# yabebalFantaye/MCEvidence

Hardware: AMD Instinct MI355X
Metric: knn_queries_per_sec (higher is better)
Workload: dtype f16 filter + f64 refine (exact f64 results)

## Files before the change

include/mcevidence_hip.h:

```cpp
#ifndef MCEVIDENCE_HIP_H
#define MCEVIDENCE_HIP_H

#include <stddef.h>
#include <stdint.h>

#ifdef __cplusplus
extern "C" {
#endif

#define MCE_ABI_VERSION 3

#define MCE_OK 0
#define MCE_ERR_INVALID (-1)
#define MCE_ERR_K_RANGE (-2)
#define MCE_ERR_HIP (-3)
#define MCE_ERR_NO_DEVICE (-4)
#define MCE_ERR_WORKSPACE (-5)
#define MCE_ERR_DIM_RANGE (-6)
#define MCE_ERR_VERIFY (-7)

#define MCE_MAX_K 32
#define MCE_MAX_DIM 63
#define MCE_GENERIC_MAX_K 1024
#define MCE_GENERIC_MAX_DIM 1024
// ... 286 lines not shown
                            double* d_fs, double* out, void* ws, size_t ws_bytes, void* stream);

int mce_set_prune_mode(int mode);
int mce_get_prune_mode(void);

int mce_set_sym_mode(int mode);
int mce_get_sym_mode(void);
int mce_last_prune_stats(double *chunk_fraction, double *tile_fraction);

void mce_set_profiling(int on);
double mce_last_kernel_ms(void);
int mce_last_search_stats(double* out, int32_t n);

int mce_debug_mfma_tile_f16(const uint16_t* yprime, const uint16_t* xprime, int32_t kst, float* out, int32_t device);
int mce_debug_mfma_tiles_f16(const uint16_t* yprime, const uint16_t* xprime, int32_t kst, int32_t ntiles, float* out, int32_t device);

#ifdef __cplusplus
}
#endif
#endif
```

mcevidence_amd/_capi.py:

```python
from __future__ import annotations

import ctypes
import os
import sys

import numpy as np

_HERE = os.path.dirname(os.path.abspath(__file__))
LIB_PATH = os.environ.get("MCE_LIB") or os.path.join(_HERE, "libmcevidence_hip.so")

MCE_OK = 0
MCE_ERR_INVALID = -1
MCE_ERR_K_RANGE = -2
MCE_ERR_HIP = -3
MCE_ERR_NO_DEVICE = -4
MCE_ERR_WORKSPACE = -5
MCE_ERR_DIM_RANGE = -6
MCE_ERR_VERIFY = -7
MCE_MAX_K = 32
MCE_MAX_DIM = 63
SELF_NONE, SELF_INCLUDE, SELF_EXCLUDE = 0, 1, 2

_c = ctypes
_P = _c.c_void_p
# ... 5 lines not shown
    "mce_last_verify_rows": (_c.c_int32, []),
    "mce_source_hash": (_c.c_char_p, []),
    "mce_release_device_memory": (None, []),
    "mce_set_search_mode": (_c.c_int, [_c.c_int]),
    "mce_get_search_mode": (_c.c_int, []),
    "mce_set_prune_mode": (_c.c_int, [_c.c_int]),
    "mce_get_prune_mode": (_c.c_int, []),
    "mce_set_sym_mode": (_c.c_int, [_c.c_int]),
    "mce_get_sym_mode": (_c.c_int, []),
    "mce_last_prune_stats": (_c.c_int, [_c.POINTER(_c.c_double), _c.POINTER(_c.c_double)]),
    "mce_set_profiling": (None, [_c.c_int]),
    "mce_last_kernel_ms": (_c.c_double, []),
    "mce_last_search_stats": (_c.c_int, [_c.c_void_p, _c.c_int32]),
    "mce_debug_mfma_tile_f16": (_c.c_int, [_P, _P, _c.c_int32, _P, _c.c_int32]),
    "mce_debug_mfma_tiles_f16": (_c.c_int, [_P, _P, _c.c_int32, _c.c_int32, _P, _c.c_int32]),
    "mce_options_push": (_c.c_int, [_P]),
    "mce_options_pop": (_c.c_int, []),
    "mce_knn_f64_opt": (_c.c_int, [_P, _c.c_int64, _P, _c.c_int64, _c.c_int32, _c.c_int32, _c.c_int32, _c.c_int64, _P, _P, _c.c_int32, _P]),
    "mce_knn_dotp_f64_opt": (_c.c_int, [_P, _c.c_int64, _P, _c.c_int64, _c.c_int32, _c.c_int32, _c.c_int32, _c.c_int64, _P, _P, _P, _P, _P, _c.c_int32, _P]),
    "mce_knn_dotp_f64_dev_opt": (_c.c_int, [_P, _c.c_int64, _P, _c.c_int64, _c.c_int32, _c.c_int32, _c.c_int32, _c.c_int64, _P, _P, _P, _P, _P, _c.c_size_t, _P, _P]),
    "mce_knn_workspace_bytes_opt": (_c.c_size_t, [_c.c_int64, _c.c_int64, _c.c_int32, _c.c_int32, _P]),
    "mce_knn_f64": (_c.c_int, [_P, _c.c_int64, _P, _c.c_int64, _c.c_int32, _c.c_int32, _c.c_int32, _c.c_int64, _P, _P, _c.c_int32]),
    "mce_dotp_f64": (_c.c_int, [_P, _c.c_int64, _c.c_int32, _c.c_int32, _c.c_int32, _c.c_int32, _P, _P, _P, _c.c_int32]),
    "mce_knn_dotp_f64": (_c.c_int, [_P, _c.c_int64, _P, _c.c_int64, _c.c_int32, _c.c_int32, _c.c_int32, _c.c_int64, _P, _P, _P, _P, _P, _c.c_int32]),
    "mce_evidence_feed_f64": (_c.c_int, [_P, _c.c_int64, _c.c_int64, _P, _c.c_int64, _c.c_int64, _c.c_int32, _c.c_int32, _c.c_int32,
                                         _P, _P, _P, _P, _P, _c.c_int32]),
    "mce_evidence_feed_part_f64": (_c.c_int, [_P, _c.c_int64, _c.c_int64, _P, _c.c_int64, _c.c_int64, _c.c_int32, _c.c_int32, _c.c_int32,
                                              _P, _P, _c.c_int32, _c.c_int32, _P, _P, _P, _P, _c.c_int32]),
    "mce_evidence_feed_whiten_f64": (_c.c_int, [_P, _c.c_int64, _c.c_int64, _c.c_int32, _c.c_int32, _P, _P, _P, _P, _P, _c.POINTER(_c.c_double), _P,
                                                _c.POINTER(_c.c_uint64), _c.c_int32]),
# ... 1112 lines not shown
    if y.shape != x.shape or y.shape[0] != 32 or y.shape[1] % 16 or not 1 <= y.shape[1] // 16 <= 8:
        raise ValueError("yprime and xprime must be float16 [32, 16*kst], kst = 1..8")
    out = np.empty((32, 32), dtype=np.float32)
    check(load().mce_debug_mfma_tile_f16(y.ctypes.data, x.ctypes.data, y.shape[1] // 16, out.ctypes.data, int(device)))
    return out


def debug_mfma_tiles(yprime, xprime, device=0):
    y = np.ascontiguousarray(yprime, dtype=np.float16)
    x = np.ascontiguousarray(xprime, dtype=np.float16)
    if y.ndim != 3 or y.shape != x.shape or y.shape[1] != 32 or y.shape[2] % 16 or not 1 <= y.shape[2] // 16 <= 8:
        raise ValueError("yprime and xprime must be float16 [ntiles, 32, 16*kst], kst = 1..8")
    out = np.empty((y.shape[0], 32, 32), dtype=np.float32)
    check(load().mce_debug_mfma_tiles_f16(y.ctypes.data, x.ctypes.data, y.shape[2] // 16, y.shape[0], out.ctypes.data, int(device)))
    return out
```

mcevidence_amd/csrc/capi_common.hpp:

```cpp
#pragma once
namespace {

thread_local char g_err[512] = "";
thread_local char g_last_kernel[256] = "";
thread_local int g_prof_on = 0;
thread_local std::vector<std::pair<hipEvent_t, hipEvent_t>> g_ev_pool;
thread_local size_t g_ev_used = 0;
thread_local size_t g_ev_calls = 0;
thread_local bool g_in_tail = false;
thread_local int g_split_depth = 0;
thread_local double g_last_prune_geom[3] = {0, 0, 0};
thread_local double g_last_flops_main = 0.0, g_last_flops_all = 0.0;
thread_local std::vector<std::pair<hipEvent_t, hipEvent_t>> g_evs_pool;
thread_local size_t g_evs_used = 0;

int fail(int code, const char* fmt, ...)
{
    va_list ap;
    va_start(ap, fmt);
    vsnprintf(g_err, sizeof(g_err), fmt, ap);
    va_end(ap);
    return code;
}

#define MCE_HIP(call)                                                                              \
    do {                                                                                           \
        hipError_t e_ = (call);                                                                    \
        if (e_ != hipSuccess)                                                                      \
            return fail(MCE_ERR_HIP, "%s failed: %s (%s:%d)", #call, hipGetErrorString(e_), __FILE__, __LINE__); \
    } while (0)

std::atomic<int> g_mode{0};
std::atomic<int> g_prune_mode{0};
struct Tuning {
    bool sym_kernel_f16 = false, tail_split = true, prune_prof = false, wide = true;
    int spin_limit = 1 << 21, sym_bucket = 0, sym_panel = 0, sym_seed_rows = 0, sym_seed_share = 2, sym_seed_mode = -1;
    int f16_seed_rows = -1, f16_seed_share = -1, f16_seed_tg = -1, rsplit = 0, panel_debug = 0, sym_chains = 0;
    size_t feed_wave_bytes = 0;
};
Tuning read_tuning()
{
    Tuning t;
    auto num = [](const char* name, int dflt) { const char* e = getenv(name); return e ? atoi(e) : dflt; };
    const char* e = getenv("MCE_SYM_KERNEL");
    t.sym_kernel_f16 = e && strcmp(e, "f16") == 0;
    t.spin_limit = num("MCE_SYM_SPIN_LIMIT", 1 << 21);
    t.sym_bucket = num("MCE_SYM_BUCKET", 0);
    t.sym_panel = num("MCE_SYM_PANEL", 0);
    t.sym_chains = num("MCE_SYM_CHAINS", 0);
    t.sym_seed_rows = num("MCE_SYM_SEED_ROWS", 0);
    t.sym_seed_share = num("MCE_SYM_SEED_SHARE", 2);
    t.sym_seed_mode = num("MCE_SYM_SEED_MODE", -1);
    t.f16_seed_rows = num("MCE_F16_SEED_ROWS", -1);
    t.f16_seed_share = num("MCE_F16_SEED_SHARE", -1);
    t.f16_seed_tg = num("MCE_F16_SEED_TG", -1);
    t.rsplit = num("MCE_RSPLIT", 0);
    t.tail_split = num("MCE_TAIL_SPLIT", 1) != 0;
    t.wide = num("MCE_WIDE", 1) != 0;
    t.panel_debug = num("MCE_PANEL_DEBUG", 0);
    t.prune_prof = getenv("MCE_PRUNE_PROF") != nullptr;
// ... 180 lines not shown
```

mcevidence_amd/csrc/capi_debug.hpp:

```cpp
#pragma once

namespace mce {
template <int KST>
__global__ __launch_bounds__(64) void mfma_tile_probe_kernel(const _Float16* __restrict__ yp, const _Float16* __restrict__ xp, float* __restrict__ out)
{
    const int lane = threadIdx.x;
    yp += (size_t)blockIdx.x * 32 * 16 * KST;
    xp += (size_t)blockIdx.x * 32 * 16 * KST;
    out += (size_t)blockIdx.x * 1024;
    v16f acc = {0.f, 0.f, 0.f, 0.f, 0.f, 0.f, 0.f, 0.f, 0.f, 0.f, 0.f, 0.f, 0.f, 0.f, 0.f, 0.f};
#pragma unroll
    for (int ks = 0; ks < KST; ++ks) {
        const v8h a = *reinterpret_cast<const v8h*>(yp + (lane & 31) * (16 * KST) + 16 * ks + 8 * (lane >> 5));
        const v8h b = *reinterpret_cast<const v8h*>(xp + (lane & 31) * (16 * KST) + 16 * ks + 8 * (lane >> 5));
        acc = __builtin_amdgcn_mfma_f32_32x32x16_f16(a, b, acc, 0, 0, 0);
    }
#pragma unroll
    for (int r = 0; r < 16; ++r) out[((r & 3) + 8 * (r >> 2) + 4 * (lane >> 5)) * 32 + (lane & 31)] = acc[r];
}
}

extern "C" int mce_debug_mfma_tiles_f16(const uint16_t* yprime, const uint16_t* xprime, int32_t kst, int32_t ntiles, float* out, int32_t device)
{
    if (!yprime || !xprime || !out) return fail(MCE_ERR_INVALID, "null pointer argument");
// ... 23 lines not shown
            case 7: hipLaunchKernelGGL(mce::mfma_tile_probe_kernel<7>, g, dim3(64), 0, nullptr, y, x, o); break;
            default: hipLaunchKernelGGL(mce::mfma_tile_probe_kernel<8>, g, dim3(64), 0, nullptr, y, x, o); break;
        }
        e = hipGetLastError();
    }
    if (e == hipSuccess) e = hipMemcpy(out, dout, (size_t)ntiles * 1024 * sizeof(float), hipMemcpyDeviceToHost);
    (void)hipFree(dy); (void)hipFree(dx); (void)hipFree(dout);
    if (e != hipSuccess) return fail(MCE_ERR_HIP, "mfma tile probe: %s", hipGetErrorString(e));
    return MCE_OK;
}

extern "C" int mce_debug_mfma_tile_f16(const uint16_t* yprime, const uint16_t* xprime, int32_t kst, float* out, int32_t device)
{
    return mce_debug_mfma_tiles_f16(yprime, xprime, kst, 1, out, device);
}
```

mcevidence_amd/csrc/capi_plan.hpp:

```cpp
#pragma once
namespace {

using mce::kMaxDevices;
constexpr int kAssumedCUs = 256;

size_t align_up(size_t x, size_t a) { return (x + a - 1) / a * a; }

constexpr bool kPruneHeavyDefault = false;
constexpr int kPruneHeavyMinBlocks = 64, kPruneHeavyCount = 700, kPruneHeavyMaxShare = 16, kPruneHeavyMinCount = 32, kPruneHeavyMaxRounds = 60;
constexpr double kPruneHeavyFullRounds = 10.0;
constexpr int kPruneHeavySplit = 4, kPruneHeavyMaxSplit = 8;
constexpr int kPruneWaveQueries = mce::kHQT * 32;
constexpr int kWideMinBlocks = 480;
bool prune_heavy_enabled()
{
    if (t_no_heavy) return false;
    const char* e = env_prune_heavy();
    return kPruneHeavyDefault || (e && *e && strcmp(e, "0") != 0);
}
static_assert(mce::kPruneWavesPerBlock == mce::kHWaves, "prune.hip orders kHWaves waves per query block");

constexpr int kRefineMargin = 2;
struct Plan {
    const mce::KnnVariant* v = nullptr;
// ... 10 lines not shown
    int64_t nrow_pad = 0;
    int nqblk = 0;
    int64_t nq_pad = 0;
    int rsplit = 1;
    int L = 4;
    size_t off_yf = 0, off_pd = 0, off_pi = 0, off_center = 0, off_msum = 0, total = 0;
    double cost = 0.0;
    int ksel = 0;
    bool twopass = false;
    bool wide_ok = false;
    bool prune = false;
    bool kd_ready = false;
    int part = 0, nparts = 1;
    int sym_qb_lo = 0, sym_qb_hi = 0;
    bool apo = false;
    int apo_phase = 0;
    int apo_nsplit = 1;
    int apo_panel = 0;
    int64_t pl_nr = 0;
    mce::PruneLayout pl;
    size_t off_prune = 0;
    size_t off_heavy = 0;
    int heavy_max = 0;
    bool sym = false;
    bool sym_active = false;
    mce::SymLayout sl;
    size_t off_sym = 0;
    int sym_nsplit = 1;
    int sym_panel = 0;
};
// ... 299 lines not shown
```

mcevidence_amd/csrc/capi_search.hpp:

```cpp
#pragma once
namespace {

double ln_unit_ball(int d) { return 0.5 * d * std::log(M_PI) - std::lgamma(1.0 + 0.5 * d); }

hipError_t launch_sym_merge(int KCAP, double* pd, int* pi, int64_t nq_pad, const mce::SymParams& sym, int qb_lo, int qb_hi, hipStream_t st, int stride = 1)
{
    const int nb = qb_hi > qb_lo ? (qb_hi - qb_lo + stride - 1) / stride : 0;
    if (nb <= 0) return hipSuccess;
    const dim3 g((unsigned)nb), b(mce::kSymMergeThreads);
    static_assert(mce::kSymMergeThreads == mce::f16_qpb(4), "one merge block per query block");
    switch (KCAP) {
        case 4: hipLaunchKernelGGL(mce::sym_merge_kernel<4>, g, b, 0, st, pd, pi, nq_pad, sym.bucket_cnt, sym.bucket_flag, sym.bucket, sym.cap, qb_lo, stride); break;
        case 8: hipLaunchKernelGGL(mce::sym_merge_kernel<8>, g, b, 0, st, pd, pi, nq_pad, sym.bucket_cnt, sym.bucket_flag, sym.bucket, sym.cap, qb_lo, stride); break;
        case 12: hipLaunchKernelGGL(mce::sym_merge_kernel<12>, g, b, 0, st, pd, pi, nq_pad, sym.bucket_cnt, sym.bucket_flag, sym.bucket, sym.cap, qb_lo, stride); break;
        default: hipLaunchKernelGGL(mce::sym_merge_kernel<16>, g, b, 0, st, pd, pi, nq_pad, sym.bucket_cnt, sym.bucket_flag, sym.bucket, sym.cap, qb_lo, stride); break;
    }
    return hipGetLastError();
}

struct KernelBracket {
    bool on = false; hipStream_t st = nullptr;
    hipError_t begin() const
    {
        if (!on) return hipSuccess;
// ... 312 lines not shown
            tiles += hi - lo;
        }
    } else {
        const double tpb = mce::kHWaves * mce::kHQT, T = (double)((nr + 31) / 32);
        for (int b = 0; b < p.nqblk; ++b) tiles += std::min(tpb * (b + 1), T);
    }
    g_last_flops_main = tiles * 16.0 * 1024.0 * 32.0 * p.KST;
    return units;
}

int Search::symmetric()
{
    char* const sw = ws + p.off_sym;
    mce::KnnF16Args a = sym_args(p, ws, nr, d, K, self_exclude);
    const Tuning tun = read_tuning();
    const int seed_rows = tun.sym_seed_rows > 0 ? tun.sym_seed_rows : (p.KST == 1 ? 65536 : 32768) * (p.apo && p.nparts >= 4 ? 2 : 1);
    const int seed_share = tun.sym_seed_share;
    auto sym_seed_for = [&](int kk) {
        int cfg = mce::f16_seed_cfg(p.nchunk, p.CT, kk + a.self_exclude, seed_rows, seed_share, MCE_H_SEED_TG);
        for (int tg = MCE_H_SEED_TG / 2; cfg == 0 && tg >= 1; tg /= 2)
            cfg = mce::f16_seed_cfg(p.nchunk, p.CT, kk + a.self_exclude, seed_rows, seed_share, tg);
        if (cfg) cfg |= ((tun.sym_seed_mode >= 0 ? tun.sym_seed_mode : kSymSeedMode[p.KST]) & 3) << 28;
        return cfg;
    };
    const int qb_lo = p.nparts > 1 && !p.apo ? (int)((int64_t)p.nqblk * p.part / p.nparts) : 0;
    const int qb_hi = p.nparts > 1 && !p.apo ? (int)((int64_t)p.nqblk * (p.part + 1) / p.nparts) : p.nqblk;
    p.sym_qb_lo = qb_lo; p.sym_qb_hi = qb_hi;
    const bool panel_kernel = !tun.sym_kernel_f16 || p.nparts > 1 || p.twopass;
    mce::PanelGeom geom;
    geom.qb_lo = qb_lo; geom.qb_hi = qb_hi; geom.tpb = mce::kHWaves * mce::kHQT; geom.ct = p.CT; geom.tpp = a.sym.panel * p.CT; geom.sym_on = 1;
    geom.ntiles = (int)((nr + 31) / 32) + (int)(((nr + 31) / 32) & 1);
// ... 21 lines not shown
        const int Kp = !p.twopass ? K : (lower ? K - 16 : 16);
        double* const pdp = pd + (lower ? list_set(p, 1) : 0);
        int* const pip = pi + (lower ? list_set(p, 1) : 0);
        if (lower) {
            MCE_HIP(mce::zero_async(a.sym.bucket_cnt, (size_t)3 * p.nqblk * sizeof(int), st));
            a.sym.slot_stride = p.KCAP;
        }
        a.ksel = lower ? K : Kp;
        a.seed_cfg = sym_seed_for(a.ksel);
        a.part_d = pdp; a.part_i = pip;
        a.qblk0 = qb_lo;
        a.nqblk_run = qb_hi - qb_lo;
        if (apo) {
            a.qblk0 = p.part; a.qblk_stride = p.nparts; a.nqblk_run = mce::apo_rank_count(p.nqblk, p.part, p.nparts);
        }
        if (a.nqblk_run > 0 && phase != 2) MCE_HIP((lower ? p.vh->launch_sym_pre32 : p.vh->launch_sym_pre)(a, st));
        a.qblk0 = 0; a.qblk_stride = 1; a.nqblk_run = 0;
        if (phase == 1) return MCE_OK;
        if (pass == 0) seed_used = a.seed_cfg;
        a.seed_cfg = 0;
        a.ksel = Kp;
        a.lo_d = lower ? pd : nullptr; a.lo_i = lower ? pi : nullptr;
        if (pass == 0) MCE_HIP(kb.begin());
        if (panel_kernel) {
            mce::PanelArgs pa;
            pa.Yh = static_cast<const _Float16*>(a.Yh); pa.Xh = static_cast<const _Float16*>(a.Xh); pa.qinfo = a.qinfo; pa.params = a.params;
            pa.X = a.X; pa.Y = a.Y; pa.rperm = a.rperm;
            pa.part_d = pdp; pa.part_i = pip; pa.nq = nq; pa.nr = nr; pa.nq_pad = p.nq_pad; pa.self_offset = 0;
            pa.D = d; pa.ksel = Kp; pa.self_exclude = a.self_exclude; pa.spin_limit = tun.spin_limit;
            pa.sym = a.sym; pa.debug = tun.panel_debug; pa.geom = geom; pa.lo_d = a.lo_d; pa.lo_i = a.lo_i;
            if (unit_table) {
                const int nun = mce::panel_unit_count(geom);
// ... 74 lines not shown
    a.ksel = p.ksel > K ? p.ksel : K;
    a.part_d = pd; a.part_i = pi;
    MCE_HIP(kb.begin());
    MCE_HIP(p.v->launch(a, st));
    MCE_HIP(kb.end());
    snprintf(g_last_kernel, sizeof(g_last_kernel), "%s grid=%d block=%d lds=%zu qt=%d ct=%d rsplit=%d", p.v->name,
             p.nqblk * p.rsplit, mce::kThreads, p.v->lds_bytes, p.QT, p.CT, p.rsplit);
    g_last_flops_main = g_last_flops_all = (double)p.nq_pad * (double)p.nrow_pad * 2.0 * 4.0 * p.KS;
    return MCE_OK;
}

int run_search(Plan& p, const double* dX, int64_t nq, const double* dY, int64_t nr, int32_t d, int32_t K,
               int32_t self_mode, int64_t self_offset, char* ws, hipStream_t st)
{
    p.sym_active = false;
    const int phase = p.apo ? p.apo_phase : 0;
    double* center = reinterpret_cast<double*>(ws + p.off_center);
    double* msum = reinterpret_cast<double*>(ws + p.off_msum);
    Search s{p, dX, nq, dY, nr, d, K, self_mode, self_offset, ws, st, phase, reinterpret_cast<double*>(ws + p.off_pd), reinterpret_cast<int*>(ws + p.off_pi),
             center, msum, (self_mode == MCE_SELF_EXCLUDE) ? 1 : 0, KernelBracket{}};
    if (p.generic) return s.generic();
    if (p.vl) {
        hipLaunchKernelGGL(mce::long_col_mean_partial_kernel, dim3(mce::kLongMeanBlocks), dim3(256), 0, st, dY, nr, (int)d, mce::kLongMeanBlocks, msum);
        MCE_HIP(hipGetLastError());
        hipLaunchKernelGGL(mce::long_col_mean_final_kernel, dim3((unsigned)((d + 255) / 256)), dim3(256), 0, st, msum, nr, (int)d, mce::kLongMeanBlocks, center);
        MCE_HIP(hipGetLastError());
    } else if (d > MCE_MAX_DIM) {
        static_assert(3 * mce::kMaxDimPad >= 128 && mce::kStatStride >= 128, "wide column means");
        hipLaunchKernelGGL(mce::col_mean_wide_partial_kernel, dim3(mce::kMeanBlocks), dim3(256), 0, st, dY, nr, (int)d, msum);
        MCE_HIP(hipGetLastError());
        hipLaunchKernelGGL(mce::col_mean_wide_final_kernel, dim3(1), dim3(128), 0, st, msum, nr, (int)d, center);
// ... 72 lines not shown
```

mcevidence_amd/csrc/knn_dispatch.hpp:

```cpp
#pragma once
#include <hip/hip_runtime.h>
#include <stdint.h>

#include "sym_types.hpp"

namespace mce {

constexpr int kMaxDevices = 64;

struct KnnArgs {
    const double* Yf;
    int64_t nchunk_total;
    int rsplit;
    const double* X;
    const double* center;
    int64_t nq;
    int D;
    int64_t nq_pad;
    int nqblk;
    int self_exclude;
    int64_t self_offset;
    int ksel;
    double* part_d;
    int* part_i;
// ... 55 lines not shown
    knn_panel_launch_fn launch_panel;
    size_t lds_bytes_panel;
    size_t lds_bytes_sym;
    int kst, kcap, qt, ct;
    size_t lds_bytes;
    const char* name;
    knn_f16_launch_fn launch_prune_short;
    int prune_short_lc;
    knn_f16_launch_fn launch_prune_short2;
    int prune_short_lc2;
    knn_f16_launch_fn launch_wide;
    size_t lds_bytes_wide;
    knn_panel_launch_fn launch_panel_lower;
    knn_f16_launch_fn launch_sym_repair_lower;
    knn_f16_launch_fn launch_sym_pre32;
};
struct DeepArgs;
typedef hipError_t (*knn_deep_launch_fn)(const DeepArgs&, hipStream_t);
struct KnnDeepVariant {
    knn_deep_launch_fn launch;
    int kst, kcap, ct;
    size_t lds_bytes;
    const char* name;
    knn_deep_launch_fn launch_lower;
};
struct LongArgs;
typedef hipError_t (*knn_long_launch_fn)(const LongArgs&, hipStream_t);
struct KnnLongVariant {
    knn_long_launch_fn launch;
    int kcap, ct;
// ... 33 lines not shown
```

mcevidence_amd/csrc/knn_inst.hip:

```cpp
#include "knn_mfma.hpp"
#include "knn_f16.hpp"
#include "knn_panel.hpp"
#include "knn_deep.hpp"
#include "knn_dispatch.hpp"

#ifndef MCE_KCAP
#error "compile with -DMCE_KCAP=n"
#endif
#ifndef MCE_INST_PART
#define MCE_INST_PART 0
#endif
#define MCE_INST_F16 (MCE_KCAP <= 16 && (MCE_INST_PART == 0 || MCE_INST_PART == 1))
#define MCE_INST_F64 (MCE_INST_PART == 0 || MCE_INST_PART == 2)
#define MCE_INST_PANEL (MCE_KCAP <= 16 && (MCE_INST_PART == 0 || MCE_INST_PART == 3))
#define MCE_INST_DEEP (MCE_KCAP <= 16 && (MCE_INST_PART == 0 || MCE_INST_PART == 4))

namespace mce {

#if MCE_INST_F64
template <int KS, int KCAP>
hipError_t launch_variant(const KnnArgs& a, hipStream_t st)
{
    constexpr size_t LDS = lds_bytes(KS, KCAP);
    static_assert(LDS <= 160 * 1024, "LDS budget");
// ... 76 lines not shown
#else
;
extern template hipError_t launch_panel_variant<1, MCE_KCAP>(const PanelArgs&, hipStream_t);
extern template hipError_t launch_panel_variant<2, MCE_KCAP>(const PanelArgs&, hipStream_t);
extern template hipError_t launch_panel_variant<3, MCE_KCAP>(const PanelArgs&, hipStream_t);
extern template hipError_t launch_panel_variant<4, MCE_KCAP>(const PanelArgs&, hipStream_t);
#if MCE_KCAP == 16
extern template hipError_t launch_panel_variant<1, MCE_KCAP, true>(const PanelArgs&, hipStream_t);
extern template hipError_t launch_panel_variant<2, MCE_KCAP, true>(const PanelArgs&, hipStream_t);
extern template hipError_t launch_panel_variant<3, MCE_KCAP, true>(const PanelArgs&, hipStream_t);
extern template hipError_t launch_panel_variant<4, MCE_KCAP, true>(const PanelArgs&, hipStream_t);
#endif
#endif
#endif

#if MCE_INST_DEEP
template <int KST, int KCAP, bool LOWER = false>
hipError_t launch_deep_variant(const DeepArgs& a, hipStream_t st)
{
    constexpr size_t LDS = deep_lds_bytes(KST);
    static_assert(LDS <= 160 * 1024, "LDS budget");
    static bool attr_set[kMaxDevices] = {};
    auto kern = knn_deep_kernel<KST, KCAP, LOWER>;
    int dev = 0;
    (void)hipGetDevice(&dev);
    if (dev >= kMaxDevices || !attr_set[dev]) {
        hipError_t e = hipFuncSetAttribute(reinterpret_cast<const void*>(kern), hipFuncAttributeMaxDynamicSharedMemorySize, (int)LDS);
        if (e != hipSuccess) return e;
        if (dev < kMaxDevices) attr_set[dev] = true;
    }
// ... 27 lines not shown
#else
#define MCE_F16_LOWER(KST) nullptr
#define MCE_F16_SYM_LOWER(KST) nullptr, nullptr, nullptr
#endif
#if MCE_KCAP == 12
#define MCE_F16_SHORT(KST) ((KST) == 1 ? &launch_f16_variant<1, MCE_KCAP, true, false, 0, 9> : (knn_f16_launch_fn) nullptr), ((KST) == 1 ? 9 : 0), \
                           ((KST) == 1 ? &launch_f16_variant<1, MCE_KCAP, true, false, 0, 10> : (knn_f16_launch_fn) nullptr), ((KST) == 1 ? 10 : 0)
#else
#define MCE_F16_SHORT(KST) nullptr, 0, nullptr, 0
#endif
#if MCE_KCAP == 4
#define MCE_F16_WIDE(KST) ((KST) == 1 ? &launch_f16_variant<1, MCE_KCAP, false, false, 0, MCE_KCAP, 4> : (knn_f16_launch_fn) nullptr), ((KST) == 1 ? f16_lds_bytes(1, MCE_KCAP, false, 4) : 0)
#else
#define MCE_F16_WIDE(KST) nullptr, 0
#endif
#define MCE_F16_VARIANT(KST, PRUNE_FN)                                                                   \
    {&launch_f16_variant<KST, MCE_KCAP, false>, PRUNE_FN, MCE_F16_LOWER(KST), &launch_f16_variant<KST, MCE_KCAP, false, false, 1>, \
     &launch_f16_variant<KST, MCE_KCAP, false, false, 2>, &launch_f16_variant<KST, MCE_KCAP, false, false, 3>, &launch_panel_variant<KST, MCE_KCAP>, panel_lds_bytes(KST), \
     f16_lds_bytes(KST, MCE_KCAP, true), KST, MCE_KCAP, f16_qt(MCE_KCAP), f16_chunk_tiles(KST), \
     f16_lds_bytes(KST, MCE_KCAP), "knn_f16_kernel<KST=" #KST ",KCAP=" MCE_STR(MCE_KCAP) ">", MCE_F16_SHORT(KST), MCE_F16_WIDE(KST), MCE_F16_SYM_LOWER(KST)}
extern const KnnF16Variant MCE_CAT(g_knn_f16_kcap, MCE_KCAP)[kMaxKST] = {
    MCE_F16_VARIANT(1, (&launch_f16_variant<1, MCE_KCAP, true>)), MCE_F16_VARIANT(2, nullptr), MCE_F16_VARIANT(3, nullptr),
    MCE_F16_VARIANT(4, nullptr),
};
#endif
#if MCE_INST_DEEP
#if MCE_KCAP == 16
#define MCE_DEEP_LOWER(KST) (&launch_deep_variant<KST, MCE_KCAP, true>)
#else
#define MCE_DEEP_LOWER(KST) nullptr
#endif
#define MCE_DEEP_VARIANT(KST) {&launch_deep_variant<KST, MCE_KCAP>, KST, MCE_KCAP, deep_chunk_tiles(KST), deep_lds_bytes(KST), "knn_deep_kernel<KST=" #KST ",KCAP=" MCE_STR(MCE_KCAP) ">", MCE_DEEP_LOWER(KST)}
extern const KnnDeepVariant MCE_CAT(g_knn_deep_kcap, MCE_KCAP)[kNumDeepKST] = {MCE_DEEP_VARIANT(5), MCE_DEEP_VARIANT(6), MCE_DEEP_VARIANT(8)};
#endif
#else
// ... 16 lines not shown
#if MCE_KCAP == 12
template __global__ void knn_f16_kernel<1, MCE_KCAP, true, false, 0, 9>(const _Float16*, int64_t, int, const _Float16*, const double*, const double*, const double*, const double*, int64_t, int64_t, int, int64_t, int, int, int64_t, int, double*, int*, const int*, const float*, int, const int*, const int*, const float*, const float*, const float*, int, int, const int*, const double*, const int*, int, SymParams, float*);
template __global__ void knn_f16_kernel<1, MCE_KCAP, true, false, 0, 10>(const _Float16*, int64_t, int, const _Float16*, const double*, const double*, const double*, const double*, int64_t, int64_t, int, int64_t, int, int, int64_t, int, double*, int*, const int*, const float*, int, const int*, const int*, const float*, const float*, const float*, int, int, const int*, const double*, const int*, int, SymParams, float*);
#endif
#if MCE_KCAP == 16
MCE_F16_INST(1, false, true, 0) MCE_F16_INST(2, false, true, 0) MCE_F16_INST(3, false, true, 0) MCE_F16_INST(4, false, true, 0)
MCE_F16_INST(1, false, true, 3) MCE_F16_INST(2, false, true, 3) MCE_F16_INST(3, false, true, 3) MCE_F16_INST(4, false, true, 3)
#define MCE_F16_INST32(KST) template __global__ void knn_f16_kernel<KST, 32, false, false, 1>(const _Float16*, int64_t, int, const _Float16*, const double*, const double*, const double*, const double*, int64_t, int64_t, int, int64_t, int, int, int64_t, int, double*, int*, const int*, const float*, int, const int*, const int*, const float*, const float*, const float*, int, int, const int*, const double*, const int*, int, SymParams, float*);
MCE_F16_INST32(1) MCE_F16_INST32(2) MCE_F16_INST32(3) MCE_F16_INST32(4)
#endif
#if MCE_KCAP == 4
template __global__ void knn_f16_kernel<1, MCE_KCAP, false, false, 0, MCE_KCAP, 4>(const _Float16*, int64_t, int, const _Float16*, const double*, const double*, const double*, const double*, int64_t, int64_t, int, int64_t, int, int, int64_t, int, double*, int*, const int*, const float*, int, const int*, const int*, const float*, const float*, const float*, int, int, const int*, const double*, const int*, int, SymParams, float*);
#endif
#endif
#if MCE_INST_PANEL
template __global__ void knn_panel_kernel<1, MCE_KCAP>(PanelArgs);
template __global__ void knn_panel_kernel<2, MCE_KCAP>(PanelArgs);
template __global__ void knn_panel_kernel<3, MCE_KCAP>(PanelArgs);
template __global__ void knn_panel_kernel<4, MCE_KCAP>(PanelArgs);
#if MCE_KCAP == 16
template __global__ void knn_panel_kernel<1, MCE_KCAP, true>(PanelArgs);
template __global__ void knn_panel_kernel<2, MCE_KCAP, true>(PanelArgs);
template __global__ void knn_panel_kernel<3, MCE_KCAP, true>(PanelArgs);
template __global__ void knn_panel_kernel<4, MCE_KCAP, true>(PanelArgs);
#endif
#endif
#if MCE_INST_F64
#define MCE_INST(KS) template __global__ void knn_mfma_kernel<KS, MCE_KCAP>(const double*, int64_t, int, const double*, const double*, int64_t, int, int64_t, int, int, int64_t, int, double*, int*);
MCE_INST(1) MCE_INST(2) MCE_INST(3) MCE_INST(4) MCE_INST(5) MCE_INST(6) MCE_INST(7) MCE_INST(8)
MCE_INST(9) MCE_INST(10) MCE_INST(11) MCE_INST(12) MCE_INST(13) MCE_INST(14) MCE_INST(15) MCE_INST(16)
// ... 6 lines not shown
```

Measured before the change: 26.88 million.

## Add dedicated seed prepass kernel for symmetric f16 sweep and raise seed rows

Introduces a new knn_seed_kernel that computes the per-query seed thresholds, row gates and tile maxima for the symmetric sweep. It uses MFMA with double-buffered LDS chunk staging and can handle two or four query tiles per wave. It becomes the default prepass, replacing the general f16 kernel in seed-only mode; the four-tile variant is picked when available. The default seed row count for KST=1 also goes up, which should tighten thresholds at the price of more seeding work. A debug entry point exposes the prepass outputs.

```diff
diff --git a/include/mcevidence_hip.h b/include/mcevidence_hip.h
--- a/include/mcevidence_hip.h
+++ b/include/mcevidence_hip.h
@@ -324,6 +324,8 @@
 
 int mce_debug_mfma_tile_f16(const uint16_t* yprime, const uint16_t* xprime, int32_t kst, float* out, int32_t device);
 int mce_debug_mfma_tiles_f16(const uint16_t* yprime, const uint16_t* xprime, int32_t kst, int32_t ntiles, float* out, int32_t device);
+int mce_debug_sym_prepass_dev(const double* dY, int64_t nr, int32_t d, int32_t K, int32_t self_mode, uint64_t* thr, uint32_t* rrow, float* rtile,
+                              int64_t cap, int64_t* nq_pad, void* ws, size_t ws_bytes, void* stream);
 
 #ifdef __cplusplus
 }
diff --git a/mcevidence_amd/_capi.py b/mcevidence_amd/_capi.py
--- a/mcevidence_amd/_capi.py
+++ b/mcevidence_amd/_capi.py
@@ -43,6 +43,7 @@
     "mce_last_search_stats": (_c.c_int, [_c.c_void_p, _c.c_int32]),
     "mce_debug_mfma_tile_f16": (_c.c_int, [_P, _P, _c.c_int32, _P, _c.c_int32]),
     "mce_debug_mfma_tiles_f16": (_c.c_int, [_P, _P, _c.c_int32, _c.c_int32, _P, _c.c_int32]),
+    "mce_debug_sym_prepass_dev": (_c.c_int, [_P, _c.c_int64, _c.c_int32, _c.c_int32, _c.c_int32, _P, _P, _P, _c.c_int64, _P, _P, _c.c_size_t, _P]),
     "mce_options_push": (_c.c_int, [_P]),
     "mce_options_pop": (_c.c_int, []),
     "mce_knn_f64_opt": (_c.c_int, [_P, _c.c_int64, _P, _c.c_int64, _c.c_int32, _c.c_int32, _c.c_int32, _c.c_int64, _P, _P, _c.c_int32, _P]),
@@ -1185,3 +1186,16 @@
     out = np.empty((y.shape[0], 32, 32), dtype=np.float32)
     check(load().mce_debug_mfma_tiles_f16(y.ctypes.data, x.ctypes.data, y.shape[2] // 16, y.shape[0], out.ctypes.data, int(device)))
     return out
+
+
+def debug_sym_prepass_dev(dY, nr, d, K, self_mode, ws, ws_bytes, stream=0):
+    lib = load()
+    npad = _c.c_int64(0)
+    check(lib.mce_debug_sym_prepass_dev(dY, int(nr), int(d), int(K), int(self_mode), None, None, None, 0, _c.addressof(npad), ws, ws_bytes, stream or None))
+    n = int(npad.value)
+    thr = np.empty(n, dtype=np.uint64)
+    rrow = np.empty(n, dtype=np.uint32)
+    rtile = np.empty(n // 32, dtype=np.float32)
+    check(lib.mce_debug_sym_prepass_dev(dY, int(nr), int(d), int(K), int(self_mode), thr.ctypes.data, rrow.ctypes.data, rtile.ctypes.data, n,
+                                        _c.addressof(npad), ws, ws_bytes, stream or None))
+    return thr, rrow, rtile
diff --git a/mcevidence_amd/csrc/capi_common.hpp b/mcevidence_amd/csrc/capi_common.hpp
--- a/mcevidence_amd/csrc/capi_common.hpp
+++ b/mcevidence_amd/csrc/capi_common.hpp
@@ -34,7 +34,7 @@
 std::atomic<int> g_prune_mode{0};
 struct Tuning {
     bool sym_kernel_f16 = false, tail_split = true, prune_prof = false, wide = true;
-    int spin_limit = 1 << 21, sym_bucket = 0, sym_panel = 0, sym_seed_rows = 0, sym_seed_share = 2, sym_seed_mode = -1;
+    int spin_limit = 1 << 21, sym_bucket = 0, sym_panel = 0, sym_seed_rows = 0, sym_seed_share = 2, sym_seed_mode = -1, sym_prepass = 0;
     int f16_seed_rows = -1, f16_seed_share = -1, f16_seed_tg = -1, rsplit = 0, panel_debug = 0, sym_chains = 0;
     size_t feed_wave_bytes = 0;
 };
@@ -44,6 +44,8 @@
     auto num = [](const char* name, int dflt) { const char* e = getenv(name); return e ? atoi(e) : dflt; };
     const char* e = getenv("MCE_SYM_KERNEL");
     t.sym_kernel_f16 = e && strcmp(e, "f16") == 0;
+    e = getenv("MCE_SYM_PREPASS");
+    t.sym_prepass = !e ? 0 : (!strcmp(e, "f16") ? 1 : (!strcmp(e, "seed2") ? 2 : (!strcmp(e, "seed4") ? 4 : 0)));
     t.spin_limit = num("MCE_SYM_SPIN_LIMIT", 1 << 21);
     t.sym_bucket = num("MCE_SYM_BUCKET", 0);
     t.sym_panel = num("MCE_SYM_PANEL", 0);
diff --git a/mcevidence_amd/csrc/capi_debug.hpp b/mcevidence_amd/csrc/capi_debug.hpp
--- a/mcevidence_amd/csrc/capi_debug.hpp
+++ b/mcevidence_amd/csrc/capi_debug.hpp
@@ -61,3 +61,31 @@
 {
     return mce_debug_mfma_tiles_f16(yprime, xprime, kst, 1, out, device);
 }
+
+extern "C" int mce_debug_sym_prepass_dev(const double* dY, int64_t nr, int32_t d, int32_t K, int32_t self_mode, uint64_t* thr, uint32_t* rrow,
+                                         float* rtile, int64_t cap, int64_t* nq_pad, void* ws, size_t ws_bytes, void* stream)
+{
+    if (!dY || !nq_pad || !ws) return fail(MCE_ERR_INVALID, "null pointer argument");
+    Plan p;
+    SameSetHint hint(true);
+    int rc = make_plan(nr, nr, d, K, self_mode, p);
+    if (rc != MCE_OK) return rc;
+    if (!p.sym || !p.vh) return fail(MCE_ERR_INVALID, "a search of this shape does not take the symmetric sweep");
+    *nq_pad = p.nq_pad;
+    if (cap == 0) return MCE_OK;
+    if (!thr || !rrow || !rtile) return fail(MCE_ERR_INVALID, "null pointer argument");
+    if (cap < p.nq_pad) return fail(MCE_ERR_INVALID, "output arrays of %lld entries, %lld needed", (long long)cap, (long long)p.nq_pad);
+    if (ws_bytes < p.total) return fail(MCE_ERR_WORKSPACE, "workspace too small: %zu < %zu", ws_bytes, p.total);
+    hipStream_t st = static_cast<hipStream_t>(stream);
+    char* wsc = static_cast<char*>(ws);
+    p.prepass_only = true;
+    rc = run_search(p, dY, nr, dY, nr, d, K, self_mode, 0, wsc, st);
+    if (rc != MCE_OK) return rc;
+    if (!p.prepass_ran) return fail(MCE_ERR_INVALID, "the search did not reach the symmetric sweep's prepass");
+    const mce::KnnF16Args a = sym_args(p, wsc, nr, d, K, self_mode == MCE_SELF_EXCLUDE ? 1 : 0);
+    MCE_HIP(hipMemcpyAsync(thr, a.sym.thr, (size_t)p.nq_pad * sizeof(uint64_t), hipMemcpyDeviceToHost, st));
+    MCE_HIP(hipMemcpyAsync(rrow, a.sym.rrow, (size_t)p.nq_pad * sizeof(uint32_t), hipMemcpyDeviceToHost, st));
+    MCE_HIP(hipMemcpyAsync(rtile, a.sym.rtile, (size_t)(p.nq_pad / 32) * sizeof(float), hipMemcpyDeviceToHost, st));
+    MCE_HIP(hipStreamSynchronize(st));
+    return MCE_OK;
+}
diff --git a/mcevidence_amd/csrc/capi_plan.hpp b/mcevidence_amd/csrc/capi_plan.hpp
--- a/mcevidence_amd/csrc/capi_plan.hpp
+++ b/mcevidence_amd/csrc/capi_plan.hpp
@@ -48,6 +48,7 @@
     int part = 0, nparts = 1;
     int sym_qb_lo = 0, sym_qb_hi = 0;
     bool apo = false;
+    bool prepass_only = false, prepass_ran = false;
     int apo_phase = 0;
     int apo_nsplit = 1;
     int apo_panel = 0;
diff --git a/mcevidence_amd/csrc/capi_search.hpp b/mcevidence_amd/csrc/capi_search.hpp
--- a/mcevidence_amd/csrc/capi_search.hpp
+++ b/mcevidence_amd/csrc/capi_search.hpp
@@ -350,7 +350,7 @@
     char* const sw = ws + p.off_sym;
     mce::KnnF16Args a = sym_args(p, ws, nr, d, K, self_exclude);
     const Tuning tun = read_tuning();
-    const int seed_rows = tun.sym_seed_rows > 0 ? tun.sym_seed_rows : (p.KST == 1 ? 65536 : 32768) * (p.apo && p.nparts >= 4 ? 2 : 1);
+    const int seed_rows = tun.sym_seed_rows > 0 ? tun.sym_seed_rows : (p.KST == 1 ? 98304 : 32768) * (p.apo && p.nparts >= 4 ? 2 : 1);
     const int seed_share = tun.sym_seed_share;
     auto sym_seed_for = [&](int kk) {
         int cfg = mce::f16_seed_cfg(p.nchunk, p.CT, kk + a.self_exclude, seed_rows, seed_share, MCE_H_SEED_TG);
@@ -402,8 +402,12 @@
         if (apo) {
             a.qblk0 = p.part; a.qblk_stride = p.nparts; a.nqblk_run = mce::apo_rank_count(p.nqblk, p.part, p.nparts);
         }
-        if (a.nqblk_run > 0 && phase != 2) MCE_HIP((lower ? p.vh->launch_sym_pre32 : p.vh->launch_sym_pre)(a, st));
+        mce::knn_f16_launch_fn pre = p.vh->launch_sym_pre4 && tun.sym_prepass != 2 ? p.vh->launch_sym_pre4 : p.vh->launch_sym_pre;
+        if (lower) pre = p.vh->launch_sym_pre32;
+        else if (tun.sym_prepass == 1) pre = p.vh->launch_sym_pre_f16;
+        if (a.nqblk_run > 0 && phase != 2) MCE_HIP(pre(a, st));
         a.qblk0 = 0; a.qblk_stride = 1; a.nqblk_run = 0;
+        p.prepass_ran = true;
         if (phase == 1) return MCE_OK;
         if (pass == 0) seed_used = a.seed_cfg;
         a.seed_cfg = 0;
@@ -508,7 +512,7 @@
                int32_t self_mode, int64_t self_offset, char* ws, hipStream_t st)
 {
     p.sym_active = false;
-    const int phase = p.apo ? p.apo_phase : 0;
+    const int phase = p.apo ? p.apo_phase : (p.prepass_only ? 1 : 0);
     double* center = reinterpret_cast<double*>(ws + p.off_center);
     double* msum = reinterpret_cast<double*>(ws + p.off_msum);
     Search s{p, dX, nq, dY, nr, d, K, self_mode, self_offset, ws, st, phase, reinterpret_cast<double*>(ws + p.off_pd), reinterpret_cast<int*>(ws + p.off_pi),
diff --git a/mcevidence_amd/csrc/knn_dispatch.hpp b/mcevidence_amd/csrc/knn_dispatch.hpp
--- a/mcevidence_amd/csrc/knn_dispatch.hpp
+++ b/mcevidence_amd/csrc/knn_dispatch.hpp
@@ -93,6 +93,8 @@
     knn_panel_launch_fn launch_panel_lower;
     knn_f16_launch_fn launch_sym_repair_lower;
     knn_f16_launch_fn launch_sym_pre32;
+    knn_f16_launch_fn launch_sym_pre_f16;
+    knn_f16_launch_fn launch_sym_pre4;
 };
 struct DeepArgs;
 typedef hipError_t (*knn_deep_launch_fn)(const DeepArgs&, hipStream_t);
diff --git a/mcevidence_amd/csrc/knn_inst.hip b/mcevidence_amd/csrc/knn_inst.hip
--- a/mcevidence_amd/csrc/knn_inst.hip
+++ b/mcevidence_amd/csrc/knn_inst.hip
@@ -1,6 +1,7 @@
 #include "knn_mfma.hpp"
 #include "knn_f16.hpp"
 #include "knn_panel.hpp"
+#include "knn_seed.hpp"
 #include "knn_deep.hpp"
 #include "knn_dispatch.hpp"
 
@@ -114,6 +115,52 @@
 #endif
 #endif
 
+#if MCE_INST_F16 || MCE_INST_PANEL
+#define MCE_SEED_WIDE (MCE_KCAP <= 12)
+#if MCE_SEED_WIDE
+#define MCE_SEED_INST4(X_) X_ template hipError_t launch_seed_variant<1, MCE_KCAP + 1, 4>(const KnnF16Args&, hipStream_t); \
+    X_ template hipError_t launch_seed_variant<2, MCE_KCAP + 1, 4>(const KnnF16Args&, hipStream_t);
+#else
+#define MCE_SEED_INST4(X_)
+#endif
+#define MCE_SEED_INST(X_) X_ template hipError_t launch_seed_variant<1, MCE_KCAP + 1, 2>(const KnnF16Args&, hipStream_t); \
+    X_ template hipError_t launch_seed_variant<2, MCE_KCAP + 1, 2>(const KnnF16Args&, hipStream_t);                         \
+    X_ template hipError_t launch_seed_variant<3, MCE_KCAP + 1, 2>(const KnnF16Args&, hipStream_t);                         \
+    X_ template hipError_t launch_seed_variant<4, MCE_KCAP + 1, 2>(const KnnF16Args&, hipStream_t);                         \
+    MCE_SEED_INST4(X_)
+template <int KST, int KSEED, int QT>
+hipError_t launch_seed_variant(const KnnF16Args& a, hipStream_t st)
+#if MCE_INST_PANEL
+{
+    constexpr size_t LDS = seed_lds_bytes(KST);
+    static_assert(LDS <= 160 * 1024, "LDS budget");
+    static bool attr_set[kMaxDevices] = {};
+    auto kern = knn_seed_kernel<KST, KSEED, QT>;
+    int dev = 0;
+    (void)hipGetDevice(&dev);
+    if (dev >= kMaxDevices || !attr_set[dev]) {
+        hipError_t e = hipFuncSetAttribute(reinterpret_cast<const void*>(kern), hipFuncAttributeMaxDynamicSharedMemorySize, (int)LDS);
+        if (e != hipSuccess) return e;
+        if (dev < kMaxDevices) attr_set[dev] = true;
+    }
+    SeedArgs s;
+    s.Yh = static_cast<const _Float16*>(a.Yh); s.Xh = static_cast<const _Float16*>(a.Xh); s.qinfo = a.qinfo; s.params = a.params;
+    s.nq = a.nq; s.nchunk_total = a.nchunk_total; s.ksel = a.ksel; s.self_exclude = a.self_exclude; s.seed_cfg = a.seed_cfg;
+    s.qblk0 = a.qblk0; s.qblk_stride = a.qblk_stride; s.nrun = a.nqblk_run ? a.nqblk_run : a.nqblk; s.kcap = KSEED - 1; s.sym = a.sym;
+    if (s.nrun <= 0) return hipSuccess;
+    constexpr int WB = QT / kHQT;
+    hipLaunchKernelGGL(kern, dim3((unsigned)((s.nrun + WB - 1) / WB)), dim3(kHThreads), LDS, st, s);
+    return hipGetLastError();
+}
+MCE_SEED_INST()
+#else
+;
+MCE_SEED_INST(extern)
+#endif
+#undef MCE_SEED_INST
+#undef MCE_SEED_INST4
+#endif
+
 #if MCE_INST_DEEP
 template <int KST, int KCAP, bool LOWER = false>
 hipError_t launch_deep_variant(const DeepArgs& a, hipStream_t st)
@@ -171,11 +218,17 @@
 #else
 #define MCE_F16_WIDE(KST) nullptr, 0
 #endif
+#if MCE_SEED_WIDE
+#define MCE_SEED_PRE4(KST) ((KST) <= 2 ? &launch_seed_variant<((KST) <= 2 ? (KST) : 1), MCE_KCAP + 1, 4> : (knn_f16_launch_fn) nullptr)
+#else
+#define MCE_SEED_PRE4(KST) nullptr
+#endif
 #define MCE_F16_VARIANT(KST, PRUNE_FN)                                                                   \
-    {&launch_f16_variant<KST, MCE_KCAP, false>, PRUNE_FN, MCE_F16_LOWER(KST), &launch_f16_variant<KST, MCE_KCAP, false, false, 1>, \
+    {&launch_f16_variant<KST, MCE_KCAP, false>, PRUNE_FN, MCE_F16_LOWER(KST), &launch_seed_variant<KST, MCE_KCAP + 1, 2>, \
      &launch_f16_variant<KST, MCE_KCAP, false, false, 2>, &launch_f16_variant<KST, MCE_KCAP, false, false, 3>, &launch_panel_variant<KST, MCE_KCAP>, panel_lds_bytes(KST), \
      f16_lds_bytes(KST, MCE_KCAP, true), KST, MCE_KCAP, f16_qt(MCE_KCAP), f16_chunk_tiles(KST), \
-     f16_lds_bytes(KST, MCE_KCAP), "knn_f16_kernel<KST=" #KST ",KCAP=" MCE_STR(MCE_KCAP) ">", MCE_F16_SHORT(KST), MCE_F16_WIDE(KST), MCE_F16_SYM_LOWER(KST)}
+     f16_lds_bytes(KST, MCE_KCAP), "knn_f16_kernel<KST=" #KST ",KCAP=" MCE_STR(MCE_KCAP) ">", MCE_F16_SHORT(KST), MCE_F16_WIDE(KST), MCE_F16_SYM_LOWER(KST), \
+     &launch_f16_variant<KST, MCE_KCAP, false, false, 1>, MCE_SEED_PRE4(KST)}
 extern const KnnF16Variant MCE_CAT(g_knn_f16_kcap, MCE_KCAP)[kMaxKST] = {
     MCE_F16_VARIANT(1, (&launch_f16_variant<1, MCE_KCAP, true>)), MCE_F16_VARIANT(2, nullptr), MCE_F16_VARIANT(3, nullptr),
     MCE_F16_VARIANT(4, nullptr),
@@ -222,6 +275,14 @@
 #endif
 #endif
 #if MCE_INST_PANEL
+template __global__ void knn_seed_kernel<1, MCE_KCAP + 1, 2>(SeedArgs);
+template __global__ void knn_seed_kernel<2, MCE_KCAP + 1, 2>(SeedArgs);
+template __global__ void knn_seed_kernel<3, MCE_KCAP + 1, 2>(SeedArgs);
+template __global__ void knn_seed_kernel<4, MCE_KCAP + 1, 2>(SeedArgs);
+#if MCE_SEED_WIDE
+template __global__ void knn_seed_kernel<1, MCE_KCAP + 1, 4>(SeedArgs);
+template __global__ void knn_seed_kernel<2, MCE_KCAP + 1, 4>(SeedArgs);
+#endif
 template __global__ void knn_panel_kernel<1, MCE_KCAP>(PanelArgs);
 template __global__ void knn_panel_kernel<2, MCE_KCAP>(PanelArgs);
 template __global__ void knn_panel_kernel<3, MCE_KCAP>(PanelArgs);
diff --git a/mcevidence_amd/csrc/knn_seed.hpp b/mcevidence_amd/csrc/knn_seed.hpp
--- /dev/null
+++ b/mcevidence_amd/csrc/knn_seed.hpp
@@ -0,0 +1,236 @@
+#pragma once
+#include "knn_f16.hpp"
+#include "knn_panel.hpp"
+
+namespace mce {
+
+struct SeedArgs {
+    const _Float16* Yh;
+    const _Float16* Xh;
+    const double* qinfo;
+    const double* params;
+    int64_t nq, nchunk_total;
+    int ksel, self_exclude;
+    int seed_cfg;
+    int qblk0, qblk_stride, nrun;
+    int kcap;
+    SymParams sym;
+};
+
+__host__ __device__ constexpr size_t seed_lds_bytes(int KST) { return (size_t)2 * f16_chunk_tiles(KST) * KST * 1024; }
+
+__device__ __forceinline__ float seed_vminf(float a, float b)
+{
+    float r;
+    asm("v_min_f32 %0, %1, %2" : "=v"(r) : "v"(a), "v"(b));
+    return r;
+}
+
+template <int KST, int KSEED, int QT>
+__global__ __launch_bounds__(kHThreads, 2) void knn_seed_kernel(SeedArgs args_by_value)
+{
+    static_assert(QT == 2 || QT == 4, "two or four query tiles per wave");
+    constexpr int NL = QT / 2;
+    constexpr int QPB = kHWaves * 64;
+    constexpr int CT = f16_chunk_tiles(KST);
+    constexpr int CHUNK_BYTES = CT * KST * 1024;
+    constexpr int VPT = CHUNK_BYTES / 16 / kHThreads;
+    static_assert(CHUNK_BYTES % (16 * kHThreads) == 0 && CT % 2 == 0, "chunk geometry");
+    (void)args_by_value;
+    typedef const __attribute__((address_space(4))) SeedArgs* ArgsPtr;
+    const ArgsPtr ap0 = (ArgsPtr)__builtin_amdgcn_kernarg_segment_ptr();
+#define MCE_SEED_ARGS() ([&]() __attribute__((always_inline)) { ArgsPtr p_ = ap0; asm volatile("" : "+s"(p_)); return p_; }())
+
+    extern __shared__ __attribute__((aligned(16))) char lds_raw[];
+    char* const stage0 = lds_raw;
+    const int tid = threadIdx.x;
+    const int lane = tid & 63;
+    const int wave = __builtin_amdgcn_readfirstlane(tid >> 6);
+    const float FINF = __builtin_huge_valf();
+
+    int64_t qbase[NL];
+    bool live[NL];
+    {
+        const ArgsPtr a = MCE_SEED_ARGS();
+        const int stride = a->qblk_stride > 1 ? a->qblk_stride : 1;
+#pragma unroll
+        for (int nl = 0; nl < NL; ++nl) {
+            const int r = (int)blockIdx.x * NL + nl;
+            live[nl] = r < a->nrun;
+            qbase[nl] = (int64_t)(a->qblk0 + (live[nl] ? r : (int)blockIdx.x * NL) * stride) * QPB + wave * 64;
+        }
+    }
+
+    v8h b[QT][KST];
+    {
+        const auto Xh = gptr(MCE_SEED_ARGS()->Xh);
+#pragma unroll
+        for (int qt = 0; qt < QT; ++qt) {
+            const int64_t q = qbase[qt >> 1] + (qt & 1) * 32 + (lane & 31);
+#pragma unroll
+            for (int ks = 0; ks < KST; ++ks) b[qt][ks] = *reinterpret_cast<const __attribute__((address_space(1))) v8h*>(Xh + q * (int64_t)(16 * KST) + 16 * ks + 8 * (lane >> 5));
+        }
+    }
+
+    int kneed, tg, nseed, nfirst;
+    int64_t cstep;
+    {
+        const ArgsPtr a = MCE_SEED_ARGS();
+        const int cfg = a->seed_cfg;
+        kneed = a->ksel + (a->self_exclude ? 1 : 0);
+        tg = (cfg >> 16) & 0xfff;
+        const int smode = (cfg >> 28) & 3;
+        const int64_t srange = a->nchunk_total;
+        nseed = ((int64_t)(cfg & 0xffff) * 2 <= srange) ? (cfg & 0xffff) : 0;
+        nfirst = smode == 1 ? nseed : (smode == 2 ? nseed / 2 : 0);
+        cstep = nseed > nfirst ? (srange - nfirst) / (nseed - nfirst) : 0;
+    }
+    const bool run = nseed > 0 && tg > 0 && kneed <= KSEED;
+    auto seed_chunk = [&](int cc) -> int64_t { return cc < nfirst ? (int64_t)cc : nfirst + (int64_t)(cc - nfirst) * cstep; };
+
+    const auto Yh_bytes = (const __attribute__((address_space(1))) char*)MCE_SEED_ARGS()->Yh;
+    auto stage_async = [&](int64_t c, int buf) { f16_stage_chunk<VPT>(Yh_bytes + c * (int64_t)CHUNK_BYTES, stage0 + buf * CHUNK_BYTES, tid, wave); };
+    auto load_a = [&](const char* lp, v8h (&a)[KST]) __attribute__((always_inline)) { f16_load_a<KST>(lp, a); };
+    auto mfma_first = [&](const v8h (&a)[KST], v16f (&acc)[QT]) __attribute__((always_inline)) {
+#pragma unroll
+        for (int qt = 0; qt < QT; ++qt) {
+            v16f z = {0.f, 0.f, 0.f, 0.f, 0.f, 0.f, 0.f, 0.f, 0.f, 0.f, 0.f, 0.f, 0.f, 0.f, 0.f, 0.f};
+            acc[qt] = __builtin_amdgcn_mfma_f32_32x32x16_f16(a[0], b[qt][0], z, 0, 0, 0);
+        }
+    };
+    auto mfma_rest = [&](const v8h (&a)[KST], v16f (&acc)[QT]) __attribute__((always_inline)) {
+#pragma unroll
+        for (int ks = 1; ks < KST; ++ks)
+#pragma unroll
+            for (int qt = 0; qt < QT; ++qt) acc[qt] = __builtin_amdgcn_mfma_f32_32x32x16_f16(a[ks], b[qt][ks], acc[qt], 0, 0, 0);
+    };
+    auto order = [&](v16f (&done)[QT], v16f (&next)[QT]) __attribute__((always_inline)) {
+#if defined(__HIP_DEVICE_COMPILE__)
+        if constexpr (QT == 2) asm volatile("" : "+v"(done[0]), "+v"(done[1]), "+v"(next[0]), "+v"(next[1]));
+        else asm volatile("" : "+v"(done[0]), "+v"(done[1]), "+v"(done[QT - 2]), "+v"(done[QT - 1]), "+v"(next[0]), "+v"(next[1]), "+v"(next[QT - 2]), "+v"(next[QT - 1]));
+#endif
+    };
+
+    float gm[QT], sm[QT][KSEED];
+#pragma unroll
+    for (int qt = 0; qt < QT; ++qt) {
+        gm[qt] = FINF;
+#pragma unroll
+        for (int k = 0; k < KSEED; ++k) sm[qt][k] = FINF;
+    }
+    int tcnt = 0;
+    auto tile_min = [&](const v16f (&acc)[QT]) __attribute__((always_inline)) {
+#pragma unroll
+        for (int qt = 0; qt < QT; ++qt) {
+            float l1[5];
+            gm[qt] = f16_min16(acc[qt], l1, gm[qt]);
+        }
+    };
+    auto group_end = [&]() __attribute__((always_inline)) {
+#pragma unroll
+        for (int qt = 0; qt < QT; ++qt) {
+            float v = seed_vminf(gm[qt], __shfl_xor(gm[qt], 32, 64));
+            gm[qt] = FINF;
+#pragma unroll
+            for (int k = 0; k < KSEED; ++k) {
+                const float lo = seed_vminf(sm[qt][k], v);
+                v = vmaxf(sm[qt][k], v);
+                sm[qt][k] = lo;
+            }
+        }
+        tcnt = 0;
+    };
+
+    if (run) {
+        v16f accA[QT], accB[QT];
+#pragma unroll
+        for (int qt = 0; qt < QT; ++qt)
+#pragma unroll
+            for (int r = 0; r < 16; ++r) accB[qt][r] = FINF;
+        const bool odd = (tg & 1) != 0;
+        auto chunk = [&](const char* lbuf) __attribute__((always_inline)) {
+            v8h a0[KST], a1[KST];
+            load_a(lbuf, a0);
+            _Pragma("unroll 1") for (int t = 0; t < CT; t += 2)
+            {
+                load_a(lbuf + ((t + 1) * KST) * 1024, a1);
+                mfma_first(a0, accA);
+                order(accB, accA);
+                mfma_rest(a0, accA);
+                tile_min(accB);
+                ++tcnt;
+                if (odd && tcnt == tg) group_end();
+                load_a(lbuf + ((t + 2 < CT ? t + 2 : t) * KST) * 1024, a0);
+                mfma_first(a1, accB);
+                order(accA, accB);
+                mfma_rest(a1, accB);
+                tile_min(accA);
+                if (++tcnt == tg) group_end();
+            }
+        };
+        stage_async(seed_chunk(0), 0);
+        for (int cc = 0; cc < nseed; ++cc) {
+            const int buf = cc & 1;
+            dma_barrier();
+            if (cc + 1 < nseed) stage_async(seed_chunk(cc + 1), buf ^ 1);
+            const char* const lbuf = stage0 + buf * CHUNK_BYTES + lane * 16;
+            chunk(lbuf);
+        }
+#if defined(__HIP_DEVICE_COMPILE__)
+        if constexpr (QT == 2) asm volatile("s_nop 15\n\ts_nop 3" : "+v"(accB[0]), "+v"(accB[1]));
+        else asm volatile("s_nop 15\n\ts_nop 3" : "+v"(accB[0]), "+v"(accB[1]), "+v"(accB[QT - 2]), "+v"(accB[QT - 1]));
+#endif
+        tile_min(accB);
+        if (++tcnt == tg) group_end();
+        if (tcnt > 0) group_end();
+    }
+
+#pragma unroll
+    for (int nl = 0; nl < NL; ++nl) {
+        float u0 = sm[2 * nl][KSEED - 1], u1 = sm[2 * nl + 1][KSEED - 1];
+#pragma unroll
+        for (int k = 0; k < KSEED - 1; ++k) {
+            u0 = (k == kneed - 1) ? sm[2 * nl][k] : u0;
+            u1 = (k == kneed - 1) ? sm[2 * nl + 1][k] : u1;
+        }
+#if defined(__HIP_DEVICE_COMPILE__)
+        asm("" : "+v"(u0), "+v"(u1));
+#endif
+        if (!live[nl]) continue;
+        const ArgsPtr a = MCE_SEED_ARGS();
+        const auto qinfo = gptr(a->qinfo);
+        const auto params = gptr(a->params);
+        const int64_t nq = a->nq;
+        const float a_up = (lane >> 5) ? u1 : u0;
+        const int64_t q = qbase[nl] + lane;
+        double thr = __builtin_huge_val();
+        if (run && q < nq && a_up < FINF) {
+            const double s2 = params[HP_SCALE] * params[HP_SCALE];
+            const double xn = qinfo[2 * q + 1];
+            const F16GateTerms t = f16_gate_terms(qinfo[2 * q], xn, params[HP_EY], params[HP_YHATMAX], params[HP_RHO], KST);
+            thr = f16_seed_bound((double)a_up, xn, t.eps, t.a, s2);
+        }
+        const auto sp_thr = gptr_w(a->sym.thr);
+        const auto sp_rrow = gptr_w(a->sym.rrow);
+        float R = 0.0f;
+        if (q < nq) {
+            sp_thr[q] = (unsigned long long)__double_as_longlong(thr);
+            R = f16_row_gate_of(thr, qinfo[2 * q], params, KST);
+            sp_rrow[q] = __float_as_uint(R);
+        } else {
+            sp_thr[q] = 0x7FF0000000000000ull;
+            sp_rrow[q] = 0u;
+        }
+        float m = R;
+#pragma unroll
+        for (int o = 16; o >= 1; o >>= 1) m = fmaxf(m, __shfl_xor(m, o, 64));
+        if ((lane & 31) == 0) gptr_w(a->sym.rtile)[q >> 5] = m;
+        const int sstride = a->sym.slot_stride ? a->sym.slot_stride : a->kcap;
+        const int64_t nrow = nq - qbase[nl] < 64 ? nq - qbase[nl] : 64;
+        const auto sl = gptr_w(a->sym.slots) + qbase[nl] * sstride;
+        for (int64_t e = lane; e < nrow * sstride; e += 64) sl[e] = 0x7FF0000000000000ull;
+    }
+#undef MCE_SEED_ARGS
+}
+
+}
```

Result: no change. 27.00 million (median of 6 runs) (+0.5%).
